# 0xPARC/plonkathon

Hardware: AMD Instinct MI355X
Metric: proofs/sec at group_order=2^11 (PLONK prover hot path: NTT + quotient + KZG MSM) (higher is better)
Workload: dtype u32x8 (254-bit Montgomery integers, BN254 Fr/Fq); 1 GPU; configs[1]: group_order=2^11, powersOfTau28_hez_final_11 SRS slice, synthetic squaring-chain witness, one distinct witness per proof; lockstep_batch=512, streams_per_gpu=20, parallelism=proof-sharded x1, ranks_in_communicator=1, gather_transport=none (single rank), msm_table_bytes=157571612672

## Files before the change

plonkathon_amd/csrc/msm_comb.h:

```cpp
#pragma once
#include <utility>

#include "msm_common.h"

#define MSM_COMB_MAX_TEETH 24
#define MSM_COMB_SEG_BITS 8
#define MSM_COMB_SCALAR_BITS 254
#define MSM_COMB_REDO 0x80000000u
PLONK_HD bool msm_comb_needs_redo(uint32_t v) { return (v & MSM_COMB_REDO) != 0 || v > MSM_DEFER_CAP; }

PLONK_HD unsigned msm_comb_columns(unsigned h) { return (MSM_COMB_SCALAR_BITS + h - 1) / h; }

struct MsmCombShape {
    unsigned h, a;
    unsigned top_bits, top_g;
    unsigned top_b;
    uint32_t top_entries;
};
PLONK_HD constexpr MsmCombShape msm_comb_shape(unsigned h, bool top) {
    MsmCombShape s{h, (MSM_COMB_SCALAR_BITS + h - 1) / h, 0, 0, 0, 0};
    if (!top) return s;
    s.a = MSM_COMB_SCALAR_BITS / h;
    s.top_bits = MSM_COMB_SCALAR_BITS - s.a * h;
    s.top_b = (2u << s.top_bits) - 1;
    s.top_entries = 1;
    while (s.top_bits && (uint64_t)s.top_entries * s.top_b <= ((uint64_t)1 << (h - 1))) {
        s.top_entries *= s.top_b;
        s.top_g++;
    }
    return s;
}
PLONK_HD constexpr bool msm_comb_top_ok(unsigned h) {
    const MsmCombShape s = msm_comb_shape(h, true);
    return h >= 2 && s.a >= 1 && s.top_bits >= 1 && s.top_bits <= 2 && s.top_g >= 1;
}
PLONK_HD size_t msm_comb_top_groups(size_t n, unsigned g) { return g ? (n + g - 1) / g : 0; }
PLONK_HD size_t msm_comb_virtual(size_t n, const MsmCombShape& s) { return s.top_g ? (msm_comb_top_groups(n, s.top_g) + s.a - 1) / s.a : 0; }
PLONK_HD size_t msm_comb_blocks(size_t n, const MsmCombShape& s) { return n + msm_comb_virtual(n, s) * s.a; }
PLONK_HD bool msm_comb_top_reach_ok(size_t n, const MsmCombShape& s) {
    return !s.top_g || ((uint64_t)(msm_comb_virtual(n, s) * (s.a - 1) + s.a) << (s.h - 1)) < ((uint64_t)1 << 31);
}
PLONK_HD size_t msm_comb_block_of(size_t i, size_t n_real, size_t top_delta) { return i + (i >= n_real ? top_delta : 0); }

struct MsmCombScale { uint32_t c[8]; };
PLONK_DEV G1Xyzz msm_comb_scaled_base(const G1Affine& P, const MsmCombScale& k) {
    G1Xyzz acc = g1_xyzz_identity();
#pragma unroll 1
    for (int bit = 255; bit >= 0; bit--) {
        g1_dbl(acc);
        if ((k.c[bit >> 5] >> (bit & 31)) & 1u) g1_madd<true>(acc, P);
    }
    return acc;
}
__global__ void __launch_bounds__(64) msm_comb_scale_kernel(const G1Affine* bases, size_t n, MsmCombScale k, G1Xyzz* out) {
    for (size_t i = (size_t)blockIdx.x * blockDim.x + threadIdx.x; i < n; i += (size_t)gridDim.x * blockDim.x) {
        G1Affine b;
        b.x = fp_load(&bases[i].x);
        b.y = fp_load(&bases[i].y);
        out[i] = msm_comb_scaled_base(b, k);
    }
}

PLONK_DEV G1Xyzz msm_comb_entry_slow(const G1Affine& P, unsigned a, unsigned h, uint32_t idx) {
    G1Xyzz acc = g1_xyzz_from_affine(P);
    const G1Affine N = g1_affine_is_identity(P) ? P : g1_affine_neg(P);
#pragma unroll 1
    for (int k = (int)h - 2; k >= 0; k--) {
#pragma unroll 1
        for (unsigned d = 0; d < a; d++) g1_dbl(acc);
        g1_madd<true>(acc, ((idx >> k) & 1) ? P : N);
    }
    return acc;
}

__global__ void msm_comb_delta_kernel(const G1Affine* cb, size_t count, G1Xyzz* out) {
    for (size_t t = (size_t)blockIdx.x * blockDim.x + threadIdx.x; t < count; t += (size_t)gridDim.x * blockDim.x) {
        G1Affine b;
        b.x = fp_load(&cb[t].x);
        b.y = fp_load(&cb[t].y);
        out[t] = g1_affine_is_identity(b) ? g1_xyzz_identity() : g1_dbl_affine(b);
    }
}

__global__ void __launch_bounds__(64) msm_comb_fill_kernel(const G1Affine* cb, const G1Affine* cd, size_t n, size_t i0, size_t nb, unsigned h,
                                                           unsigned sb, G1Xyzz* tmp) {
    const size_t nseg = (size_t)1 << (h - 1 - sb), seg_len = (size_t)1 << sb;
    for (size_t id = (size_t)blockIdx.x * blockDim.x + threadIdx.x; id < nb * nseg; id += (size_t)gridDim.x * blockDim.x) {
        const size_t bi = id / nseg, i = i0 + bi, idx0 = (id % nseg) << sb;
        G1Affine t;
        t.x = fp_load(&cb[(size_t)(h - 1) * n + i].x);
        t.y = fp_load(&cb[(size_t)(h - 1) * n + i].y);
        G1Xyzz acc = g1_xyzz_from_affine(t);
#pragma unroll 1
        for (unsigned k = 0; k + 1 < h; k++) {
            t.x = fp_load(&cb[(size_t)k * n + i].x);
            t.y = fp_load(&cb[(size_t)k * n + i].y);
            if (!((idx0 >> k) & 1)) t.y = fp_neg(t.y);
            g1_madd<true>(acc, t);
        }
        G1Xyzz* out = tmp + (bi << (h - 1)) + idx0;
        out[0] = acc;
#pragma unroll 1
        for (uint32_t s = 1; s < seg_len; s++) {
            const unsigned b = (unsigned)__builtin_ctz(s);
            const uint32_t gray = s ^ (s >> 1);
            t.x = fp_load(&cd[(size_t)b * n + i].x);
            t.y = fp_load(&cd[(size_t)b * n + i].y);
            if (!((gray >> b) & 1)) t.y = fp_neg(t.y);
            g1_madd<true>(acc, t);
            out[gray] = acc;
        }
    }
}

__global__ void __launch_bounds__(64) msm_comb_top_base_kernel(const G1Affine* pb, size_t n, unsigned L, unsigned a, unsigned g, G1Xyzz* out) {
    for (size_t i = (size_t)blockIdx.x * blockDim.x + threadIdx.x; i < n; i += (size_t)gridDim.x * blockDim.x) {
        G1Affine b;
        b.x = fp_load(&pb[i].x);
        b.y = fp_load(&pb[i].y);
        G1Xyzz p = g1_xyzz_from_affine(b);
        const unsigned j = (unsigned)((i / g) % a);
#pragma unroll 1
        for (unsigned k = 0; k < L - j; k++) g1_dbl(p);
        out[i] = p;
    }
}
PLONK_DEV G1Affine msm_comb_top_point(const G1Affine* tq, size_t n, size_t i, bool neg) {
    G1Affine q = g1_affine_identity();
    if (i < n) {
        q.x = fp_load(&tq[i].x);
        q.y = fp_load(&tq[i].y);
        if (neg && !g1_affine_is_identity(q)) q.y = fp_neg(q.y);
    }
    return q;
}
__global__ void __launch_bounds__(64) msm_comb_top_fill_kernel(const G1Affine* tq, size_t n, size_t g0, size_t ng, unsigned hb, unsigned g, unsigned B,
                                                               uint32_t entries, G1Xyzz* tmp) {
    const unsigned low = g >= 2 ? 2u : 1u, run = low == 2 ? B * B : B, c = (B - 1) / 2;
    const size_t runs = entries / run;
    for (size_t id = (size_t)blockIdx.x * blockDim.x + threadIdx.x; id < ng * runs; id += (size_t)gridDim.x * blockDim.x) {
        const size_t bi = id / runs, grp = g0 + bi, i0 = grp * g;
        uint32_t t = (uint32_t)(id - bi * runs);
        G1Xyzz* out = tmp + (bi << hb) + (size_t)t * run;
        G1Xyzz acc = g1_xyzz_identity();
#pragma unroll 1
        for (unsigned pos = low; pos < g; pos++) {
            const int code = (int)(t % B) - (int)c;
            t /= B;
            const G1Affine q = msm_comb_top_point(tq, n, i0 + pos, code < 0);
#pragma unroll 1
            for (int k = 0; k < (code < 0 ? -code : code); k++) g1_madd<true>(acc, q);
        }
        const G1Affine q0 = msm_comb_top_point(tq, n, i0, false), m0 = msm_comb_top_point(tq, n, i0, true);
        const G1Affine q1 = msm_comb_top_point(tq, n, low == 2 ? i0 + 1 : n, false), m1 = msm_comb_top_point(tq, n, low == 2 ? i0 + 1 : n, true);
#pragma unroll 1
        for (unsigned k = 0; k < c; k++) {
            g1_madd<true>(acc, m0);
            g1_madd<true>(acc, m1);
        }
#pragma unroll 1
        for (unsigned d1 = 0; d1 < (low == 2 ? B : 1u); d1++) {
            const bool down = (d1 & 1u) != 0;
#pragma unroll 1
            for (unsigned st = 0; st < B; st++) {
                out[d1 * B + (down ? B - 1 - st : st)] = acc;
                if (st + 1 < B) g1_madd<true>(acc, down ? m0 : q0);
            }
            if (d1 + 1 < B) g1_madd<true>(acc, q1);
        }
    }
}

template <unsigned H, bool TOP> __global__ void __launch_bounds__(256) msm_comb_digits_kernel(const Fr* scalars, size_t n, size_t stride, size_t inner,
                                                                                              size_t outer_stride, size_t m0, uint32_t* digits, size_t nd) {
    constexpr MsmCombShape SH = msm_comb_shape(H, TOP);
    constexpr unsigned A = SH.a, L = A * H;
    static_assert(L <= 9 * 32 && H <= MSM_COMB_MAX_TEETH, "the recoded scalar is kept in nine words");
    constexpr unsigned PER = TOP ? (256 / (SH.top_g ? SH.top_g : 1)) * (SH.top_g ? SH.top_g : 1) : 256;
    const size_t m = m0 + blockIdx.y, i = (size_t)blockIdx.x * PER + threadIdx.x;
    const bool live = threadIdx.x < PER && i < n;
    int code = 0;
    if (live) {
        const Fr* sc = msm_scalar_row(scalars, m, stride, inner, outer_stride);
        const Fr s = fp_load(sc + i);
        const bool even = !(s.v[0] & 1u);
        uint32_t sp[8], br = 0;
#pragma unroll
        for (int k = 0; k < 8; k++) {
            const uint32_t d = fp_sbb(FrParams::mod(k), s.v[k], br);
            sp[k] = even ? d : s.v[k];
        }
        uint32_t w[9];
#pragma unroll
        for (int k = 0; k < 8; k++) w[k] = (sp[k] >> 1) | (k < 7 ? sp[k + 1] << 31 : 0u);
        w[8] = 0;
        if constexpr (TOP) {
            constexpr unsigned hi = L >> 5, sh = L & 31;
            uint32_t u = sp[hi] >> sh;
            if constexpr (sh + SH.top_bits > 32 && hi + 1 < 8) u |= sp[hi + 1] << (32 - sh);
            code = (int)(u & ((1u << SH.top_bits) - 1u));
            if (even) code = -code;
#pragma unroll
            for (unsigned k = 0; k < 9; k++) {
                if (k > ((L - 1) >> 5)) w[k] = 0;
                else if (k == ((L - 1) >> 5)) w[k] &= (1u << ((L - 1) & 31)) - 1u;
            }
        }
        w[(L - 1) >> 5] |= 1u << ((L - 1) & 31);
        uint32_t* out = digits + (m * A) * nd + i;
#pragma unroll
        for (unsigned j = 0; j < A; j++) {
            uint32_t idx = 0;
#pragma unroll
            for (unsigned k = 0; k < H; k++) {
                const unsigned p = j + A * k;
                idx |= ((w[p >> 5] >> (p & 31)) & 1u) << k;
            }
            const uint32_t top = idx >> (H - 1), mask = (1u << (H - 1)) - 1u;
            const uint32_t low = top ? (idx & mask) : (~idx & mask);
            const uint32_t neg = (top ? 0u : 1u) ^ (even ? 1u : 0u);
            out[(size_t)j * nd] = low | (neg << 31);
        }
    }
    if constexpr (TOP) {
        constexpr unsigned G = SH.top_g, B = SH.top_b;
        __shared__ int codes[256];
        codes[threadIdx.x] = code;
        __syncthreads();
        const size_t grp = (size_t)blockIdx.x * (PER / G) + threadIdx.x, nv = msm_comb_virtual(n, SH);
        if (threadIdx.x < PER / G && grp < nv * A) {
            uint32_t idx = 0, pw = 1;
#pragma unroll
            for (unsigned pos = 0; pos < G; pos++) {
                idx += (uint32_t)(codes[threadIdx.x * G + pos] + (int)((B - 1) / 2)) * pw;
                pw *= B;
            }
            const size_t v = grp / A, j = grp - v * A;
            digits[(m * A + j) * nd + n + v] = (uint32_t)((v * (A - 1) + j) << (H - 1)) + idx;
        }
    }
}

struct MsmCombPlan {
    uint32_t q, p, n_main, n_left;
};
PLONK_HD MsmCombPlan msm_comb_plan(uint32_t nsub, uint32_t a) {
    MsmCombPlan pl;
    pl.q = MSM_BLOCK / a;
    pl.p = (a * nsub + MSM_BLOCK - 1) / MSM_BLOCK;
    const uint32_t reach = pl.q * pl.p;
    pl.n_main = reach < nsub ? reach : nsub;
    pl.n_left = nsub - pl.n_main;
    return pl;
}
PLONK_HD void msm_comb_left_pieces(const MsmCombPlan& pl, uint32_t j, uint32_t& ulo, uint32_t& x) {
    if (!pl.n_left) {
        ulo = 0;
        x = 0;
        return;
    }
    ulo = (j * pl.n_left) / pl.p;
    x = ((j + 1) * pl.n_left - 1) / pl.p - ulo + 1;
}
PLONK_HD uint32_t msm_comb_slot(const MsmCombPlan& pl, uint32_t a, uint32_t j, uint32_t r, uint32_t ulo) {
    return r < pl.q ? j * pl.q + r : a * pl.q + ulo + j + (r - pl.q);
}

__global__ void __launch_bounds__(MSM_BLOCK, MSM_ACC_WAVES) msm_comb_kernel(const G1Affine* lookup, unsigned hb, unsigned a,
                                                                             const uint32_t* digits, size_t n, unsigned G,
                                                                             G1Xyzz* partial, MsmDeferred* deferred, size_t deferred_stride,
                                                                             uint32_t* n_deferred, unsigned n_real, unsigned top_delta) {
    PLONK_DYN_SMEM(smem);
    G1Xyzz* red = reinterpret_cast<G1Xyzz*>(smem);
    const unsigned m = blockIdx.x / G, g = blockIdx.x % G, tid = threadIdx.x;
    const uint32_t per_g = (uint32_t)((n + G - 1) / G);
    const uint32_t s0 = g * per_g < n ? g * per_g : (uint32_t)n, s1 = s0 + per_g < n ? s0 + per_g : (uint32_t)n, nsub = s1 - s0;
    const MsmCombPlan pl = msm_comb_plan(nsub, a);
    const uint32_t* dg = digits + (size_t)m * a * n + s0;
    const G1Affine* tab = lookup + ((size_t)s0 << hb);
    const uint32_t nr_rel = n_real > s0 ? n_real - s0 : 0u;
    uint32_t j, i, step, count, slot;
    const bool column_lane = tid < a * pl.q;
    if (column_lane) {
        j = tid / pl.q;
        i = tid - j * pl.q;
        step = pl.q;
        count = i < pl.n_main ? (pl.n_main - 1 - i) / pl.q + 1 : 0;
        slot = tid;
    } else {
        const uint32_t u = tid - a * pl.q, items = a * pl.n_left;
        const uint32_t lo = u * pl.p < items ? u * pl.p : items, hi = lo + pl.p < items ? lo + pl.p : items;
        count = hi - lo;
        j = pl.n_left ? lo / pl.n_left : 0;
        i = pl.n_main + (lo - j * pl.n_left);
        step = 1;
        slot = a * pl.q + u + j;
    }
    G1XyzzL run = g1l_identity();
    auto flush = [&]() { red[slot] = g1l_to_piece(run); };
    for (uint32_t k = 0; k < count; k++) {
        const uint32_t d = dg[(size_t)j * n + i];
        const G1Affine* src = tab + (((size_t)(i + (i >= nr_rel ? top_delta : 0u)) << hb) + (d & 0x7fffffffu));
        const Fq x = fp_load(&src->x), y = fp_load(&src->y);
        if (!g1l_madd_fast(run, x, y, (d >> 31) != 0) && !(fp_is_zero(x) && fp_is_zero(y))) {
            const uint32_t sl = atomicAdd(n_deferred + m, 1u);
            if (sl < MSM_DEFER_CAP) deferred[(size_t)m * deferred_stride + sl] = MsmDeferred{(uint32_t)(j * n + s0 + i), d};
        }
        i += step;
        if (i >= nsub && k + 1 < count) {
            flush();
            run = g1l_identity();
            slot++;
            j++;
            i = pl.n_main;
        }
    }
    if (column_lane || count) flush();
    __syncthreads();
    uint32_t cur = pl.q + (pl.n_left ? (pl.n_left + pl.p - 1) / pl.p + 1 : 0);
    while (cur > 1) {
        const uint32_t half = (cur + 1) / 2, cnt = cur - half;
        for (uint32_t w = tid; w < a * cnt; w += MSM_BLOCK) {
            const uint32_t jj = w / cnt, r = w - jj * cnt;
            uint32_t ulo, x;
            msm_comb_left_pieces(pl, jj, ulo, x);
            if (r + half < pl.q + x) {
                const uint32_t sa = msm_comb_slot(pl, a, jj, r, ulo), sb = msm_comb_slot(pl, a, jj, r + half, ulo);
                const G1XyzzL o = g1l_from_piece(&red[sb]);
                if (!o.inf) {
                    G1XyzzL v = g1l_from_piece(&red[sa]);
                    if (!g1l_add_fast(v, o)) atomicOr(n_deferred + m, MSM_COMB_REDO);
                    red[sa] = g1l_to_piece_wide(v);
                }
            }
        }
        __syncthreads();
        cur = half;
    }
    if (tid < a) partial[((size_t)m * G + g) * a + tid] = red[tid * pl.q];
}

__global__ void __launch_bounds__(64) msm_comb_colsum_kernel(const G1Xyzz* partial, unsigned G, unsigned a, G1Xyzz* colsum, uint32_t* n_deferred) {
    const size_t m = blockIdx.x / a, j = blockIdx.x % a;
    const unsigned lane = threadIdx.x;
    G1XyzzL acc = g1l_identity();
    bool ok = true;
    for (unsigned g = lane; g < G; g += 64) ok &= g1l_add_fast(acc, g1l_from_piece(&partial[(m * G + g) * a + j]));
    ok &= g1l_wave_reduce_step<32>(acc, lane);
    ok &= g1l_wave_reduce_step<16>(acc, lane);
    ok &= g1l_wave_reduce_step<8>(acc, lane);
    ok &= g1l_wave_reduce_step<4>(acc, lane);
    ok &= g1l_wave_reduce_step<2>(acc, lane);
    ok &= g1l_wave_reduce_step<1>(acc, lane);
    if (!ok) atomicOr(n_deferred + m, MSM_COMB_REDO);
    if (lane == 0) colsum[m * a + j] = g1l_to_piece_wide(acc);
}

template <unsigned LPM> __global__ void __launch_bounds__(64) msm_comb_finalize_kernel(const G1Xyzz* sums, size_t M, unsigned G, unsigned a,
                                                                                       const G1Affine* lookup, unsigned hb, size_t n,
                                                                                       const MsmDeferred* deferred, size_t deferred_stride,
                                                                                       uint32_t* n_deferred, Fq* out_xy, uint8_t* flags, unsigned n_real,
                                                                                       unsigned top_delta) {
    const size_t gid = (size_t)blockIdx.x * 64 + threadIdx.x, m = gid / LPM;
    const unsigned l = (unsigned)(gid % LPM), lane = threadIdx.x;
    G1XyzzL acc = g1l_identity();
    bool ok = true;
    if (m < M && l < a) {
        const uint32_t nd = msm_comb_needs_redo(n_deferred[m]) ? 0u : n_deferred[m];
        const unsigned jtop = l + ((a - 1 - l) / LPM) * LPM;
#pragma unroll 1
        for (int j = (int)jtop; j >= 0; j -= (int)LPM) {
            if (j != (int)jtop)
#pragma unroll 1
                for (unsigned d = 0; d < LPM; d++) g1l_dbl(acc);
#pragma unroll 1
            for (unsigned g = 0; g < G; g++) ok &= g1l_add_fast<true>(acc, g1l_from_piece(&sums[(m * G + g) * a + j]));
#pragma unroll 1
            for (uint32_t k = 0; k < nd; k++) {
                const MsmDeferred e = deferred[m * deferred_stride + k];
                if (e.bucket / n != (uint32_t)j) continue;
                const size_t i = e.bucket - (size_t)j * n;
                const G1Affine* src = lookup + ((msm_comb_block_of(i, n_real, top_delta) << hb) + (e.entry & 0x7fffffffu));
                const Fq x = fp_load(&src->x), y = fp_load(&src->y);
                if (!(fp_is_zero(x) && fp_is_zero(y))) ok &= g1l_madd_fast(acc, x, y, (e.entry >> 31) != 0);
            }
        }
#pragma unroll 1
        for (unsigned d = 0; d < l; d++) g1l_dbl(acc);
    }
    if constexpr (LPM >= 2) ok &= g1l_wave_reduce_step<1, true>(acc, lane);
    if constexpr (LPM >= 4) ok &= g1l_wave_reduce_step<2, true>(acc, lane);
    if constexpr (LPM >= 8) ok &= g1l_wave_reduce_step<4, true>(acc, lane);
    if constexpr (LPM >= 16) ok &= g1l_wave_reduce_step<8, true>(acc, lane);
    if constexpr (LPM >= 32) ok &= g1l_wave_reduce_step<16, true>(acc, lane);
    if constexpr (LPM >= 64) ok &= g1l_wave_reduce_step<32, true>(acc, lane);
    if (m < M && !ok) atomicOr(n_deferred + m, MSM_COMB_REDO);
    if (m < M && l == 0) msm_store_result(g1l_to_xyzz(acc), m, out_xy, flags);
}

__global__ void __launch_bounds__(256) msm_comb_slow_kernel(const G1Affine* lookup, unsigned hb, unsigned a, const uint32_t* digits, size_t n,
                                                            const uint32_t* n_deferred, Fq* out_xy, uint8_t* flags, unsigned n_real, unsigned top_delta) {
    __shared__ G1Xyzz red[256];
    const unsigned m = blockIdx.x, tid = threadIdx.x;
    if (!msm_comb_needs_redo(n_deferred[m])) return;
    const uint32_t* dg = digits + (size_t)m * a * n;
    G1Xyzz acc = g1_xyzz_identity();
#pragma unroll 1
    for (int j = (int)a - 1; j >= 0; j--) {
        g1_dbl(acc);
#pragma unroll 1
        for (size_t i = tid; i < n; i += 256) {
            const uint32_t d = dg[(size_t)j * n + i];
            const G1Affine* src = lookup + ((msm_comb_block_of(i, n_real, top_delta) << hb) + (d & 0x7fffffffu));
            G1Affine pt;
            pt.x = fp_load(&src->x);
            pt.y = fp_load(&src->y);
            if (d >> 31) pt.y = fp_neg(pt.y);
            g1_madd<true>(acc, pt);
        }
    }
    msm_fold_store(red, acc, tid, 256, m, out_xy, flags);
}

PLONK_DEV bool msm_comb_entry_matches(const G1Affine& P0, const MsmCombScale& k, unsigned a, unsigned h, uint32_t idx, const G1Affine* e) {
    const G1Affine P = g1_to_affine(msm_comb_scaled_base(P0, k));
    const G1Xyzz v = msm_comb_entry_slow(P, a, h, idx);
    const Fq ex = fp_load(&e->x), ey = fp_load(&e->y);
    if (g1_is_identity(v)) return fp_is_zero(ex) && fp_is_zero(ey);
    return fp_eq(fp_mul(ex, v.zz), v.x) && fp_eq(fp_mul(ey, v.zzz), v.y);
}
__global__ void __launch_bounds__(64) msm_comb_verify_kernel(const G1Affine* bases, const G1Affine* lookup, size_t n, unsigned a, unsigned h,
                                                             unsigned samples, MsmCombScale k, unsigned* mismatches) {
    const size_t t = (size_t)blockIdx.x * blockDim.x + threadIdx.x;
    if (t >= n + 2 * (size_t)samples) return;
    const uint32_t mask = (1u << (h - 1)) - 1u;
    size_t i;
    uint32_t idx;
    if (t < n) {
        i = t;
        idx = mask;
    } else {
        const unsigned s = (unsigned)(t - n) >> 1;
        i = n <= samples ? (s < n ? s : n - 1) : (size_t)s * (n - 1) / (samples - 1);
        idx = ((t - n) & 1) ? (0x55555555u & mask) : 0u;
    }
    G1Affine b;
    b.x = fp_load(&bases[i].x);
    b.y = fp_load(&bases[i].y);
    if (!msm_comb_entry_matches(b, k, a, h, idx, lookup + ((i << (h - 1)) + idx))) atomicAdd(mismatches, 1u);
}

__global__ void __launch_bounds__(64) msm_comb_verify_top_kernel(const G1Affine* bases, const G1Affine* lookup, size_t n, unsigned a, unsigned h, unsigned g,
                                                                 unsigned B, MsmCombScale k, unsigned* mismatches) {
    const size_t grp = (size_t)blockIdx.x * blockDim.x + threadIdx.x;
    if (grp >= msm_comb_top_groups(n, g)) return;
    const unsigned L = a * h, j = (unsigned)(grp % a);
    G1Xyzz sum = g1_xyzz_identity();
    uint32_t idx = 0, pw = 1;
#pragma unroll 1
    for (unsigned pos = 0; pos < g; pos++, pw *= B) {
        const size_t i = grp * g + pos;
        idx += ((B - 1) / 2 + (i < n ? 1u : 0u)) * pw;
        if (i >= n) continue;
        G1Affine b;
        b.x = fp_load(&bases[i].x);
        b.y = fp_load(&bases[i].y);
        G1Xyzz p = msm_comb_scaled_base(b, k);
#pragma unroll 1
        for (unsigned d = 0; d < L - j; d++) g1_dbl(p);
        g1_add(sum, p);
    }
    const G1Affine* e = lookup + (((n + grp) << (h - 1)) + idx);
    const Fq ex = fp_load(&e->x), ey = fp_load(&e->y);
    const bool ok = g1_is_identity(sum) ? (fp_is_zero(ex) && fp_is_zero(ey)) : (fp_eq(fp_mul(ex, sum.zz), sum.x) && fp_eq(fp_mul(ey, sum.zzz), sum.y));
    if (!ok) atomicAdd(mismatches, 1u);
}

static size_t msm_comb_stage_entries(size_t n, unsigned h) {
    const size_t half = (size_t)1 << (h - 1);
    size_t bases = n / 8 ? n / 8 : 1;
    while (bases > 1 && bases * half > ((size_t)1 << 27)) bases /= 2;
    return bases * half;
}
static size_t msm_comb_bytes(size_t n, unsigned h, bool top) {
    return (msm_comb_blocks(n, msm_comb_shape(h, top)) << (h - 1)) * sizeof(G1Affine) + msm_comb_stage_entries(n, h) * sizeof(G1Xyzz);
}
static double msm_comb_additions(unsigned h, bool top) {
    const MsmCombShape sh = msm_comb_shape(h, top);
    return (double)sh.a + (top ? 1.0 / sh.top_g : 0.0);
}
bool msm_comb_takes_top(unsigned teeth) { return teeth >= 2 && teeth <= MSM_COMB_MAX_TEETH && msm_comb_top_ok(teeth); }
static bool msm_comb_takes_top_for(size_t n, unsigned h) { return msm_comb_top_ok(h) && msm_comb_top_reach_ok(n, msm_comb_shape(h, true)); }
static bool msm_comb_well_formed(const MsmLookupTable* t) {
    if (t->bits < 2 || t->bits > MSM_COMB_MAX_TEETH) return false;
    const bool top = t->top_g != 0;
    if (top && !msm_comb_top_ok(t->bits)) return false;
    const MsmCombShape sh = msm_comb_shape(t->bits, top);
    return t->windows == sh.a && t->top_bits == sh.top_bits && t->top_g == sh.top_g &&
           t->bytes == (msm_comb_blocks(t->n_points, sh) << (t->bits - 1)) * sizeof(G1Affine);
}

static MsmCombScale msm_comb_scale_constant() {
    Fr one_plain = fp_zero<FrParams>();
    one_plain.v[0] = 1;
    const Fr c = fp_from_mont(one_plain);
    MsmCombScale k;
    for (int i = 0; i < 8; i++) k.c[i] = c.v[i];
    return k;
}

static int msm_comb_build(plonk_ctx* ctx, const plonk_srs* srs, unsigned h, bool top, MsmLookupTable* t) {
    if (top && !msm_comb_top_ok(h)) {
        plonk_set_error("a comb of %u teeth takes no top tables (254 mod teeth must be 1 or 2)", h);
        return PLONK_ERR_ARG;
    }
    const MsmCombShape sh = msm_comb_shape(h, top);
    if (!msm_comb_top_reach_ok(srs->n_points, sh)) {
        plonk_set_error("%zu bases are too many for the top tables of a %u-tooth comb (a virtual scalar's block offset must fit 31 bits)", srs->n_points, h);
        return PLONK_ERR_ARG;
    }
    const unsigned a = sh.a, sb = h - 1 < MSM_COMB_SEG_BITS ? h - 1 : MSM_COMB_SEG_BITS;
    const size_t n = srs->n_points, half = (size_t)1 << (h - 1), stage = msm_comb_stage_entries(n, h), chunk_bases = stage / half;
    const size_t blocks = msm_comb_blocks(n, sh);
    void *gx = nullptr, *gb = nullptr, *dx = nullptr, *db = nullptr, *tmp = nullptr, *tab = nullptr, *pb = nullptr;
    auto fail = [&]() {
        for (void* q : {gx, gb, dx, db, tmp, tab, pb})
            if (q) hipFree(q);
        (void)hipGetLastError();
        plonk_set_error("the %u-tooth comb table (%zu MiB) does not fit in device memory", h, msm_comb_bytes(n, h, top) >> 20);
        return PLONK_ERR_NOMEM;
    };
    if (!plonk_dev_malloc(&tab, blocks * half * sizeof(G1Affine))) return fail();
    if (!plonk_dev_malloc(&tmp, stage * sizeof(G1Xyzz))) return fail();
    if (!plonk_dev_malloc(&gx, n * h * sizeof(G1Xyzz))) return fail();
    if (!plonk_dev_malloc(&gb, n * h * sizeof(G1Affine))) return fail();
    if (!plonk_dev_malloc(&dx, n * (sb ? sb : 1) * sizeof(G1Xyzz))) return fail();
    if (!plonk_dev_malloc(&db, n * (sb ? sb : 1) * sizeof(G1Affine))) return fail();
    if (!plonk_dev_malloc(&pb, n * sizeof(G1Affine))) return fail();
    PLONK_LAUNCH(msm_comb_scale_kernel, grid1(n, 64, 2048), dim3(64), 0, ctx->stream, (const G1Affine*)srs->bases, n, msm_comb_scale_constant(), (G1Xyzz*)gx);
    g1_batch_to_affine(ctx, (const G1Xyzz*)gx, (G1Affine*)pb, n);
    msm_window_bases(ctx, (const G1Affine*)pb, n, a, h, (G1Xyzz*)gx);
    g1_batch_to_affine(ctx, (const G1Xyzz*)gx, (G1Affine*)gb, n * h);
    if (sb) {
        PLONK_LAUNCH(msm_comb_delta_kernel, grid1(n * sb), dim3(256), 0, ctx->stream, (const G1Affine*)gb, n * sb, (G1Xyzz*)dx);
        g1_batch_to_affine(ctx, (const G1Xyzz*)dx, (G1Affine*)db, n * sb);
    }
    for (size_t i0 = 0; i0 < n; i0 += chunk_bases) {
        const size_t nb = n - i0 < chunk_bases ? n - i0 : chunk_bases, lanes = nb << (h - 1 - sb);
        PLONK_LAUNCH(msm_comb_fill_kernel, grid1(lanes, 64, 65536), dim3(64), 0, ctx->stream, (const G1Affine*)gb, (const G1Affine*)db, n, i0, nb, h, sb,
                     (G1Xyzz*)tmp);
        g1_batch_to_affine(ctx, (const G1Xyzz*)tmp, (G1Affine*)tab + i0 * half, nb * half);
    }
    if (top) {
        PLONK_LAUNCH(msm_comb_top_base_kernel, grid1(n, 64, 2048), dim3(64), 0, ctx->stream, (const G1Affine*)pb, n, a * h, a, sh.top_g, (G1Xyzz*)gx);
        g1_batch_to_affine(ctx, (const G1Xyzz*)gx, (G1Affine*)gb, n);
        const size_t groups = msm_comb_top_groups(n, sh.top_g), vblocks = blocks - n, run = sh.top_g >= 2 ? (size_t)sh.top_b * sh.top_b : sh.top_b;
        for (size_t g0 = 0; g0 < vblocks; g0 += chunk_bases) {
            const size_t nb = vblocks - g0 < chunk_bases ? vblocks - g0 : chunk_bases;
            const size_t ng = g0 >= groups ? 0 : (groups - g0 < nb ? groups - g0 : nb);
            if (hipMemsetAsync(tmp, 0, nb * half * sizeof(G1Xyzz), ctx->stream) != hipSuccess) return fail();
            if (ng)
                PLONK_LAUNCH(msm_comb_top_fill_kernel, grid1(ng * (sh.top_entries / run), 64, 65536), dim3(64), 0, ctx->stream, (const G1Affine*)gb, n, g0, ng,
                             h - 1, sh.top_g, sh.top_b, sh.top_entries, (G1Xyzz*)tmp);
            g1_batch_to_affine(ctx, (const G1Xyzz*)tmp, (G1Affine*)tab + (n + g0) * half, nb * half);
        }
    }
    if (hipGetLastError() != hipSuccess || hipStreamSynchronize(ctx->stream) != hipSuccess) return fail();
    for (void* q : {gx, gb, dx, db, tmp, pb}) hipFree(q);
    t->kind = MSM_TABLE_COMB;
    t->bits = h;
    t->windows = a;
    t->top_bits = sh.top_bits;
    t->top_g = sh.top_g;
    t->data = (G1Affine*)tab;
    t->bytes = blocks * half * sizeof(G1Affine);
    return PLONK_OK;
}

static void msm_comb_verify(plonk_ctx* ctx, const plonk_srs* srs, const MsmLookupTable* t, unsigned* d_mismatches) {
    const size_t lanes = srs->n_points + 2 * LUT_VERIFY_SAMPLES;
    PLONK_LAUNCH(msm_comb_verify_kernel, dim3((unsigned)((lanes + 63) / 64)), dim3(64), 0, ctx->stream, (const G1Affine*)srs->bases,
                 (const G1Affine*)t->data, srs->n_points, t->windows, t->bits, (unsigned)LUT_VERIFY_SAMPLES, msm_comb_scale_constant(), d_mismatches);
    if (t->top_g) {
        const size_t groups = msm_comb_top_groups(srs->n_points, t->top_g);
        PLONK_LAUNCH(msm_comb_verify_top_kernel, dim3((unsigned)((groups + 63) / 64)), dim3(64), 0, ctx->stream, (const G1Affine*)srs->bases,
                     (const G1Affine*)t->data, srs->n_points, t->windows, t->bits, t->top_g, (2u << t->top_bits) - 1u, msm_comb_scale_constant(),
                     d_mismatches);
    }
}

template <unsigned H, bool TOP> static void msm_comb_launch_digits(plonk_ctx* ctx, const Fr* d_scalars, size_t n, size_t stride, size_t inner,
                                                                   size_t outer_stride, size_t M, uint32_t* digits, size_t nd) {
    if constexpr (!TOP || msm_comb_top_ok(H)) {
        constexpr MsmCombShape SH = msm_comb_shape(H, TOP);
        constexpr unsigned G = TOP ? SH.top_g : 1, PER = (256 / G) * G;
        size_t gx = (n + PER - 1) / PER;
        if (TOP) {
            const size_t gv = ((nd - n) * SH.a + PER / G - 1) / (PER / G);
            gx = gx > gv ? gx : gv;
        }
        void (*kern)(const Fr*, size_t, size_t, size_t, size_t, size_t, uint32_t*, size_t) = msm_comb_digits_kernel<H, TOP>;
        for (size_t m0 = 0; m0 < M; m0 += 32768) {
            const size_t rows = M - m0 < 32768 ? M - m0 : 32768;
            PLONK_LAUNCH(kern, dim3((unsigned)gx, (unsigned)rows), dim3(256), 0, ctx->stream, d_scalars, n, stride, inner,
                         outer_stride, m0, digits, nd);
        }
    }
}
typedef void (*msm_comb_digits_fn)(plonk_ctx*, const Fr*, size_t, size_t, size_t, size_t, size_t, uint32_t*, size_t);
template <bool TOP, unsigned... H> static msm_comb_digits_fn msm_comb_digits_for(unsigned h, std::integer_sequence<unsigned, H...>) {
    msm_comb_digits_fn fn = nullptr;
    ((h == H + 2 && (!TOP || msm_comb_top_ok(H + 2)) ? (void)(fn = &msm_comb_launch_digits<H + 2, TOP>) : (void)0), ...);
    return fn;
}

static int msm_run_comb(plonk_ctx* ctx, const plonk_srs* srs, const Fr* d_scalars, size_t n_real, size_t M, size_t stride, Fq* d_out_xy, uint8_t* d_flags,
                        size_t inner, size_t outer_stride) {
    const G1Affine* table = srs->shared->data;
    const unsigned h = srs->shared->bits, a = srs->shared->windows, hb = h - 1;
    const bool top = srs->shared->top_g != 0;
    const MsmCombShape sh = msm_comb_shape(h, top);
    const size_t nv = msm_comb_virtual(n_real, sh), n = n_real + nv;
    const unsigned top_delta = (unsigned)(srs->n_points - n_real);
    PLONK_REQUIRE((uint64_t)n * a < ((uint64_t)1 << 32), PLONK_ERR_ARG, "MSM size %zu too large for the lookup path", n_real);
    PLONK_REQUIRE(msm_comb_top_reach_ok(n_real, sh), PLONK_ERR_ARG, "MSM size %zu too large for the top tables of %u teeth", n_real, h);
    unsigned G = msm_groups_per_msm(ctx, M, 64, 3072 / (MSM_BLOCK / 64), 0.035, n * a, 2);
    while (G > 1 && (size_t)G > n) G /= 2;
    MsmScratch s;
    const size_t part_off = s.take(M * G * a * sizeof(G1Xyzz)), col_off = s.take(G >= 4 ? M * a * sizeof(G1Xyzz) : 0), cnt_off = s.take(M * 4);
    const size_t dfr_off = s.take(M * MSM_DEFER_CAP * sizeof(MsmDeferred)), dig_off = s.take(M * a * n * 4);
    PLONK_TRY(ctx_scratch(ctx, 1, s.total, (void**)&s.base));
    G1Xyzz *partial = s.at<G1Xyzz>(part_off), *colsum = s.at<G1Xyzz>(col_off);
    uint32_t *n_deferred = s.at<uint32_t>(cnt_off), *digits = s.at<uint32_t>(dig_off);
    MsmDeferred* deferred = s.at<MsmDeferred>(dfr_off);
    const auto teeth = std::make_integer_sequence<unsigned, MSM_COMB_MAX_TEETH - 1>();
    const msm_comb_digits_fn digits_fn = top ? msm_comb_digits_for<true>(h, teeth) : msm_comb_digits_for<false>(h, teeth);
    PLONK_REQUIRE(digits_fn, PLONK_ERR_ARG, "no comb of %u teeth", h);
    PLONK_CHECK_HIP(hipMemsetAsync(n_deferred, 0, M * 4, ctx->stream));
    PLONK_TRY(prof_begin(ctx, "msm_digits", (double)M * (double)n * (32.0 + 4.0 * a)));
    digits_fn(ctx, d_scalars, n_real, stride, inner, outer_stride, M, digits, n);
    PLONK_TRY(prof_end(ctx));
    const size_t lds = (size_t)(MSM_BLOCK + a) * sizeof(G1Xyzz);
    PLONK_TRY(prof_begin(ctx, "msm_comb", (double)M * (96.0 * (double)n_real + 64.0)));
    PLONK_LAUNCH(msm_comb_kernel, dim3((unsigned)(M * G)), dim3(MSM_BLOCK), lds, ctx->stream, table, hb, a, (const uint32_t*)digits, n, G, partial,
                 deferred, (size_t)MSM_DEFER_CAP, n_deferred, (unsigned)n_real, top_delta);
    PLONK_TRY(prof_end(ctx));
    const G1Xyzz* sums = partial;
    unsigned Gf = G;
    if (G >= 4) {
        PLONK_LAUNCH(msm_comb_colsum_kernel, dim3((unsigned)(M * a)), dim3(64), 0, ctx->stream, (const G1Xyzz*)partial, G, a, colsum, n_deferred);
        sums = colsum;
        Gf = 1;
    }
#define PLONK_COMB_FINALIZE(L)                                                                                                                      \
    PLONK_LAUNCH(msm_comb_finalize_kernel<L>, dim3((unsigned)((M * L + 63) / 64)), dim3(64), 0, ctx->stream, sums, M, Gf, a, table, hb, n,            \
                 (const MsmDeferred*)deferred, (size_t)MSM_DEFER_CAP, n_deferred, d_out_xy, d_flags, (unsigned)n_real, top_delta)
    if (M >= 64) PLONK_COMB_FINALIZE(4);
    else PLONK_COMB_FINALIZE(16);
#undef PLONK_COMB_FINALIZE
    PLONK_LAUNCH(msm_comb_slow_kernel, dim3((unsigned)M), dim3(256), 0, ctx->stream, table, hb, a, (const uint32_t*)digits, n, (const uint32_t*)n_deferred,
                 d_out_xy, d_flags, (unsigned)n_real, top_delta);
    PLONK_CHECK_HIP(hipGetLastError());
    return PLONK_OK;
}

static const MsmTableLayout msm_comb_layout = {22,
                                               msm_comb_takes_top_for,
                                               msm_comb_additions,
                                               msm_comb_bytes,
                                               msm_comb_well_formed,
                                               msm_comb_build,
                                               msm_comb_verify,
                                               msm_run_comb};
```

Measured before the change: 48480 proofs/s.

## Batch comb MSM: spill pieces to global, add pieces reducer, table-driven digit recoding

```diff
diff --git a/plonkathon_amd/csrc/msm_comb.h b/plonkathon_amd/csrc/msm_comb.h
--- a/plonkathon_amd/csrc/msm_comb.h
+++ b/plonkathon_amd/csrc/msm_comb.h
@@ -171,14 +171,33 @@
     }
 }
 
+PLONK_HD constexpr bool msm_comb_digits_by_table(unsigned a) { return a <= 13; }
+struct alignas(8) MsmCombSpread { uint32_t lo, hi; };
+PLONK_HD constexpr uint32_t msm_comb_spread8(uint32_t v) {
+    uint32_t x = v & 0xffu;
+    x = (x | (x << 12)) & 0x000f000fu;
+    x = (x | (x << 6)) & 0x03030303u;
+    return (x | (x << 3)) & 0x11111111u;
+}
 template <unsigned H, bool TOP> __global__ void __launch_bounds__(256) msm_comb_digits_kernel(const Fr* scalars, size_t n, size_t stride, size_t inner,
-                                                                                              size_t outer_stride, size_t m0, uint32_t* digits, size_t nd) {
+                                                                                              size_t outer_stride, size_t m0, uint32_t* digits, size_t nd,
+                                                                                              uint32_t* n_deferred) {
     constexpr MsmCombShape SH = msm_comb_shape(H, TOP);
     constexpr unsigned A = SH.a, L = A * H;
     static_assert(L <= 9 * 32 && H <= MSM_COMB_MAX_TEETH, "the recoded scalar is kept in nine words");
     constexpr unsigned PER = TOP ? (256 / (SH.top_g ? SH.top_g : 1)) * (SH.top_g ? SH.top_g : 1) : 256;
+    constexpr bool TABLE = msm_comb_digits_by_table(A);
     const size_t m = m0 + blockIdx.y, i = (size_t)blockIdx.x * PER + threadIdx.x;
     const bool live = threadIdx.x < PER && i < n;
+    if (blockIdx.x == 0 && threadIdx.x == 0) n_deferred[m] = 0;
+    __shared__ MsmCombSpread spread[TABLE ? 1u << A : 1u];
+    if constexpr (TABLE) {
+        const uint32_t lo = msm_comb_spread8(threadIdx.x);
+#pragma unroll
+        for (unsigned e = 0; e < ((1u << A) + 255) / 256; e++)
+            if (threadIdx.x + 256 * e < (1u << A)) spread[threadIdx.x + 256 * e] = MsmCombSpread{lo, msm_comb_spread8(e)};
+        __syncthreads();
+    }
     int code = 0;
     if (live) {
         const Fr* sc = msm_scalar_row(scalars, m, stride, inner, outer_stride);
@@ -208,13 +227,35 @@
         }
         w[(L - 1) >> 5] |= 1u << ((L - 1) & 31);
         uint32_t* out = digits + (m * A) * nd + i;
+        uint32_t nib[TABLE ? (H + 3) / 4 : 1][2];
+        if constexpr (TABLE) {
+#pragma unroll
+            for (unsigned g = 0; g < (H + 3) / 4; g++) {
+                nib[g][0] = nib[g][1] = 0;
+#pragma unroll
+                for (unsigned c = 0; c < 4 && 4 * g + c < H; c++) {
+                    constexpr uint32_t cmask = (1u << A) - 1u;
+                    const unsigned p = A * (4 * g + c), lw = p >> 5, sh = p & 31;
+                    uint32_t ch = w[lw] >> sh;
+                    if (sh + A > 32) ch |= w[lw + 1] << (32 - sh);
+                    const MsmCombSpread e = spread[ch & cmask];
+                    nib[g][0] |= e.lo << c;
+                    nib[g][1] |= e.hi << c;
+                }
+            }
+        }
 #pragma unroll
         for (unsigned j = 0; j < A; j++) {
             uint32_t idx = 0;
-#pragma unroll
-            for (unsigned k = 0; k < H; k++) {
-                const unsigned p = j + A * k;
-                idx |= ((w[p >> 5] >> (p & 31)) & 1u) << k;
+            if constexpr (TABLE) {
+#pragma unroll
+                for (unsigned g = 0; g < (H + 3) / 4; g++) idx |= ((nib[g][j >> 3] >> (4 * (j & 7))) & 15u) << (4 * g);
+            } else {
+#pragma unroll
+                for (unsigned k = 0; k < H; k++) {
+                    const unsigned p = j + A * k;
+                    idx |= ((w[p >> 5] >> (p & 31)) & 1u) << k;
+                }
             }
             const uint32_t top = idx >> (H - 1), mask = (1u << (H - 1)) - 1u;
             const uint32_t low = top ? (idx & mask) : (~idx & mask);
@@ -266,12 +307,13 @@
     return r < pl.q ? j * pl.q + r : a * pl.q + ulo + j + (r - pl.q);
 }
 
+template <bool BATCH>
 __global__ void __launch_bounds__(MSM_BLOCK, MSM_ACC_WAVES) msm_comb_kernel(const G1Affine* lookup, unsigned hb, unsigned a,
                                                                              const uint32_t* digits, size_t n, unsigned G,
                                                                              G1Xyzz* partial, MsmDeferred* deferred, size_t deferred_stride,
                                                                              uint32_t* n_deferred, unsigned n_real, unsigned top_delta) {
     PLONK_DYN_SMEM(smem);
-    G1Xyzz* red = reinterpret_cast<G1Xyzz*>(smem);
+    G1Xyzz* red = BATCH ? partial + (size_t)blockIdx.x * (MSM_BLOCK + a) : reinterpret_cast<G1Xyzz*>(smem);
     const unsigned m = blockIdx.x / G, g = blockIdx.x % G, tid = threadIdx.x;
     const uint32_t per_g = (uint32_t)((n + G - 1) / G);
     const uint32_t s0 = g * per_g < n ? g * per_g : (uint32_t)n, s1 = s0 + per_g < n ? s0 + per_g : (uint32_t)n, nsub = s1 - s0;
@@ -316,6 +358,7 @@
         }
     }
     if (column_lane || count) flush();
+    if constexpr (BATCH) return;
     __syncthreads();
     uint32_t cur = pl.q + (pl.n_left ? (pl.n_left + pl.p - 1) / pl.p + 1 : 0);
     while (cur > 1) {
@@ -356,6 +399,35 @@
     if (lane == 0) colsum[m * a + j] = g1l_to_piece_wide(acc);
 }
 
+#ifndef MSM_COMB_SUM_LANES
+#define MSM_COMB_SUM_LANES 1
+#endif
+template <unsigned LPC> __global__ void __launch_bounds__(64) msm_comb_pieces_kernel(const G1Xyzz* pieces, size_t M, unsigned G, unsigned a, size_t n,
+                                                                                     G1Xyzz* colsum, uint32_t* n_deferred) {
+    const size_t gid = (size_t)blockIdx.x * 64 + threadIdx.x, col = gid / LPC, m = col / a;
+    const unsigned l = (unsigned)(gid % LPC), j = (unsigned)(col - m * a), lane = threadIdx.x;
+    G1XyzzL acc = g1l_identity();
+    bool ok = true;
+    if (m < M) {
+        const uint32_t per_g = (uint32_t)((n + G - 1) / G);
+#pragma unroll 1
+        for (unsigned g = 0; g < G; g++) {
+            const uint32_t s0 = g * per_g < n ? g * per_g : (uint32_t)n, s1 = s0 + per_g < n ? s0 + per_g : (uint32_t)n;
+            const MsmCombPlan pl = msm_comb_plan(s1 - s0, a);
+            uint32_t ulo, x;
+            msm_comb_left_pieces(pl, j, ulo, x);
+            const G1Xyzz* src = pieces + (m * G + g) * (MSM_BLOCK + a);
+#pragma unroll 1
+            for (uint32_t r = l; r < pl.q + x; r += LPC) ok &= g1l_add_fast(acc, g1l_from_piece(&src[msm_comb_slot(pl, a, j, r, ulo)]));
+        }
+    }
+    if constexpr (LPC >= 2) ok &= g1l_wave_reduce_step<1>(acc, lane);
+    if constexpr (LPC >= 4) ok &= g1l_wave_reduce_step<2>(acc, lane);
+    if constexpr (LPC >= 8) ok &= g1l_wave_reduce_step<4>(acc, lane);
+    if (m < M && !ok) atomicOr(n_deferred + m, MSM_COMB_REDO);
+    if (m < M && l == 0) colsum[m * a + j] = g1l_to_piece_wide(acc);
+}
+
 template <unsigned LPM> __global__ void __launch_bounds__(64) msm_comb_finalize_kernel(const G1Xyzz* sums, size_t M, unsigned G, unsigned a,
                                                                                        const G1Affine* lookup, unsigned hb, size_t n,
                                                                                        const MsmDeferred* deferred, size_t deferred_stride,
@@ -398,28 +470,46 @@
     if (m < M && l == 0) msm_store_result(g1l_to_xyzz(acc), m, out_xy, flags);
 }
 
-__global__ void __launch_bounds__(256) msm_comb_slow_kernel(const G1Affine* lookup, unsigned hb, unsigned a, const uint32_t* digits, size_t n,
+__global__ void __launch_bounds__(256) msm_comb_slow_kernel(const G1Affine* lookup, unsigned hb, unsigned a, const uint32_t* digits, size_t n, size_t M,
                                                             const uint32_t* n_deferred, Fq* out_xy, uint8_t* flags, unsigned n_real, unsigned top_delta) {
     __shared__ G1Xyzz red[256];
-    const unsigned m = blockIdx.x, tid = threadIdx.x;
-    if (!msm_comb_needs_redo(n_deferred[m])) return;
-    const uint32_t* dg = digits + (size_t)m * a * n;
-    G1Xyzz acc = g1_xyzz_identity();
-#pragma unroll 1
-    for (int j = (int)a - 1; j >= 0; j--) {
-        g1_dbl(acc);
-#pragma unroll 1
-        for (size_t i = tid; i < n; i += 256) {
-            const uint32_t d = dg[(size_t)j * n + i];
-            const G1Affine* src = lookup + ((msm_comb_block_of(i, n_real, top_delta) << hb) + (d & 0x7fffffffu));
-            G1Affine pt;
-            pt.x = fp_load(&src->x);
-            pt.y = fp_load(&src->y);
-            if (d >> 31) pt.y = fp_neg(pt.y);
-            g1_madd<true>(acc, pt);
-        }
-    }
-    msm_fold_store(red, acc, tid, 256, m, out_xy, flags);
+    const unsigned tid = threadIdx.x;
+#pragma unroll 1
+    for (size_t m = blockIdx.x; m < M; m += gridDim.x) {
+        if (!msm_comb_needs_redo(n_deferred[m])) continue;
+        const uint32_t* dg = digits + m * a * n;
+        G1Xyzz acc = g1_xyzz_identity();
+#pragma unroll 1
+        for (int j = (int)a - 1; j >= 0; j--) {
+            g1_dbl(acc);
+#pragma unroll 1
+            for (size_t i = tid; i < n; i += 256) {
+                const uint32_t d = dg[(size_t)j * n + i];
+                const G1Affine* src = lookup + ((msm_comb_block_of(i, n_real, top_delta) << hb) + (d & 0x7fffffffu));
+                G1Affine pt;
+                pt.x = fp_load(&src->x);
+                pt.y = fp_load(&src->y);
+                if (d >> 31) pt.y = fp_neg(pt.y);
+                g1_madd<true>(acc, pt);
+            }
+        }
+        red[tid] = acc;
+        __syncthreads();
+        for (unsigned s = 128; s >= 64; s >>= 1) {
+            if (tid < s) {
+                G1Xyzz x = red[tid];
+                g1_add(x, red[tid + s]);
+                red[tid] = x;
+            }
+            __syncthreads();
+        }
+        if (tid < 64) {
+            G1Xyzz total = red[tid];
+            g1_wave_reduce(total, tid);
+            if (tid == 0) msm_store_result(total, m, out_xy, flags);
+        }
+        __syncthreads();
+    }
 }
 
 PLONK_DEV bool msm_comb_entry_matches(const G1Affine& P0, const MsmCombScale& k, unsigned a, unsigned h, uint32_t idx, const G1Affine* e) {
@@ -590,7 +680,7 @@
 }
 
 template <unsigned H, bool TOP> static void msm_comb_launch_digits(plonk_ctx* ctx, const Fr* d_scalars, size_t n, size_t stride, size_t inner,
-                                                                   size_t outer_stride, size_t M, uint32_t* digits, size_t nd) {
+                                                                   size_t outer_stride, size_t M, uint32_t* digits, size_t nd, uint32_t* n_deferred) {
     if constexpr (!TOP || msm_comb_top_ok(H)) {
         constexpr MsmCombShape SH = msm_comb_shape(H, TOP);
         constexpr unsigned G = TOP ? SH.top_g : 1, PER = (256 / G) * G;
@@ -599,15 +689,15 @@
             const size_t gv = ((nd - n) * SH.a + PER / G - 1) / (PER / G);
             gx = gx > gv ? gx : gv;
         }
-        void (*kern)(const Fr*, size_t, size_t, size_t, size_t, size_t, uint32_t*, size_t) = msm_comb_digits_kernel<H, TOP>;
+        void (*kern)(const Fr*, size_t, size_t, size_t, size_t, size_t, uint32_t*, size_t, uint32_t*) = msm_comb_digits_kernel<H, TOP>;
         for (size_t m0 = 0; m0 < M; m0 += 32768) {
             const size_t rows = M - m0 < 32768 ? M - m0 : 32768;
             PLONK_LAUNCH(kern, dim3((unsigned)gx, (unsigned)rows), dim3(256), 0, ctx->stream, d_scalars, n, stride, inner,
-                         outer_stride, m0, digits, nd);
-        }
-    }
-}
-typedef void (*msm_comb_digits_fn)(plonk_ctx*, const Fr*, size_t, size_t, size_t, size_t, size_t, uint32_t*, size_t);
+                         outer_stride, m0, digits, nd, n_deferred);
+        }
+    }
+}
+typedef void (*msm_comb_digits_fn)(plonk_ctx*, const Fr*, size_t, size_t, size_t, size_t, size_t, uint32_t*, size_t, uint32_t*);
 template <bool TOP, unsigned... H> static msm_comb_digits_fn msm_comb_digits_for(unsigned h, std::integer_sequence<unsigned, H...>) {
     msm_comb_digits_fn fn = nullptr;
     ((h == H + 2 && (!TOP || msm_comb_top_ok(H + 2)) ? (void)(fn = &msm_comb_launch_digits<H + 2, TOP>) : (void)0), ...);
@@ -626,8 +716,10 @@
     PLONK_REQUIRE(msm_comb_top_reach_ok(n_real, sh), PLONK_ERR_ARG, "MSM size %zu too large for the top tables of %u teeth", n_real, h);
     unsigned G = msm_groups_per_msm(ctx, M, 64, 3072 / (MSM_BLOCK / 64), 0.035, n * a, 2);
     while (G > 1 && (size_t)G > n) G /= 2;
+    const bool batch = M >= 64;
     MsmScratch s;
-    const size_t part_off = s.take(M * G * a * sizeof(G1Xyzz)), col_off = s.take(G >= 4 ? M * a * sizeof(G1Xyzz) : 0), cnt_off = s.take(M * 4);
+    const size_t part_off = s.take(M * G * (batch ? MSM_BLOCK + a : a) * sizeof(G1Xyzz));
+    const size_t col_off = s.take(batch || G >= 4 ? M * a * sizeof(G1Xyzz) : 0), cnt_off = s.take(M * 4);
     const size_t dfr_off = s.take(M * MSM_DEFER_CAP * sizeof(MsmDeferred)), dig_off = s.take(M * a * n * 4);
     PLONK_TRY(ctx_scratch(ctx, 1, s.total, (void**)&s.base));
     G1Xyzz *partial = s.at<G1Xyzz>(part_off), *colsum = s.at<G1Xyzz>(col_off);
@@ -636,18 +728,26 @@
     const auto teeth = std::make_integer_sequence<unsigned, MSM_COMB_MAX_TEETH - 1>();
     const msm_comb_digits_fn digits_fn = top ? msm_comb_digits_for<true>(h, teeth) : msm_comb_digits_for<false>(h, teeth);
     PLONK_REQUIRE(digits_fn, PLONK_ERR_ARG, "no comb of %u teeth", h);
-    PLONK_CHECK_HIP(hipMemsetAsync(n_deferred, 0, M * 4, ctx->stream));
     PLONK_TRY(prof_begin(ctx, "msm_digits", (double)M * (double)n * (32.0 + 4.0 * a)));
-    digits_fn(ctx, d_scalars, n_real, stride, inner, outer_stride, M, digits, n);
-    PLONK_TRY(prof_end(ctx));
-    const size_t lds = (size_t)(MSM_BLOCK + a) * sizeof(G1Xyzz);
-    PLONK_TRY(prof_begin(ctx, "msm_comb", (double)M * (96.0 * (double)n_real + 64.0)));
-    PLONK_LAUNCH(msm_comb_kernel, dim3((unsigned)(M * G)), dim3(MSM_BLOCK), lds, ctx->stream, table, hb, a, (const uint32_t*)digits, n, G, partial,
-                 deferred, (size_t)MSM_DEFER_CAP, n_deferred, (unsigned)n_real, top_delta);
+    digits_fn(ctx, d_scalars, n_real, stride, inner, outer_stride, M, digits, n, n_deferred);
     PLONK_TRY(prof_end(ctx));
     const G1Xyzz* sums = partial;
     unsigned Gf = G;
-    if (G >= 4) {
+    PLONK_TRY(prof_begin(ctx, "msm_comb", (double)M * (96.0 * (double)n_real + 64.0)));
+    if (batch) {
+        PLONK_LAUNCH(msm_comb_kernel<true>, dim3((unsigned)(M * G)), dim3(MSM_BLOCK), 0, ctx->stream, table, hb, a, (const uint32_t*)digits, n, G, partial,
+                     deferred, (size_t)MSM_DEFER_CAP, n_deferred, (unsigned)n_real, top_delta);
+        PLONK_LAUNCH(msm_comb_pieces_kernel<MSM_COMB_SUM_LANES>, dim3((unsigned)((M * a * MSM_COMB_SUM_LANES + 63) / 64)), dim3(64), 0, ctx->stream,
+                     (const G1Xyzz*)partial, M, G, a, n, colsum, n_deferred);
+        sums = colsum;
+        Gf = 1;
+    } else {
+        const size_t lds = (size_t)(MSM_BLOCK + a) * sizeof(G1Xyzz);
+        PLONK_LAUNCH(msm_comb_kernel<false>, dim3((unsigned)(M * G)), dim3(MSM_BLOCK), lds, ctx->stream, table, hb, a, (const uint32_t*)digits, n, G, partial,
+                     deferred, (size_t)MSM_DEFER_CAP, n_deferred, (unsigned)n_real, top_delta);
+    }
+    PLONK_TRY(prof_end(ctx));
+    if (!batch && G >= 4) {
         PLONK_LAUNCH(msm_comb_colsum_kernel, dim3((unsigned)(M * a)), dim3(64), 0, ctx->stream, (const G1Xyzz*)partial, G, a, colsum, n_deferred);
         sums = colsum;
         Gf = 1;
@@ -655,11 +755,11 @@
 #define PLONK_COMB_FINALIZE(L)                                                                                                                      \
     PLONK_LAUNCH(msm_comb_finalize_kernel<L>, dim3((unsigned)((M * L + 63) / 64)), dim3(64), 0, ctx->stream, sums, M, Gf, a, table, hb, n,            \
                  (const MsmDeferred*)deferred, (size_t)MSM_DEFER_CAP, n_deferred, d_out_xy, d_flags, (unsigned)n_real, top_delta)
-    if (M >= 64) PLONK_COMB_FINALIZE(4);
+    if (batch) PLONK_COMB_FINALIZE(4);
     else PLONK_COMB_FINALIZE(16);
 #undef PLONK_COMB_FINALIZE
-    PLONK_LAUNCH(msm_comb_slow_kernel, dim3((unsigned)M), dim3(256), 0, ctx->stream, table, hb, a, (const uint32_t*)digits, n, (const uint32_t*)n_deferred,
-                 d_out_xy, d_flags, (unsigned)n_real, top_delta);
+    PLONK_LAUNCH(msm_comb_slow_kernel, dim3((unsigned)(M < 64 ? M : 64)), dim3(256), 0, ctx->stream, table, hb, a, (const uint32_t*)digits, n, M,
+                 (const uint32_t*)n_deferred, d_out_xy, d_flags, (unsigned)n_real, top_delta);
     PLONK_CHECK_HIP(hipGetLastError());
     return PLONK_OK;
 }
```

Result: slower. 47930 proofs/s (-1.1%).
